# QueensGambit/CrazyAra

Measured on AMD Instinct MI355X. Metric: nn_evals_per_sec, higher is better.
Workload: dtype f16x3; 1 GPU; crazyhouse RISEv2 19-block (34x8x8 planes -> 5184 policy + value), batch=256, inputs resident in HBM, random-init seeded weights; batch=256, parallelism=replicas x1, precision=float16x3

## Files before the change

### crazyara_amd/csrc/nn/kernels.h

```cpp
#pragma once
#include <hip/hip_runtime.h>
#include <cstdint>

namespace cra {

typedef _Float16 half_t;

constexpr int kSquares = 64;

inline int64_t packed_weight_elems(int cout_pad, int k_total) { return int64_t(cout_pad) * k_total; }

struct ConvArgs {
    const void* x;
    const void* wpk;
    const void* wpk_lo;
    const float* bias;
    const void* resid;
    void* out;
    int batch;
    int cin;
    int cout_pad;
    int cout_real;
    int cout_ld;
    int ks;
    int relu;
    int out_policy_f32;
    int out_flat;
    int flat_pitch;
    int out_rows_f32;
    int rows_valid;
    float* softmax_out;
    const float* planes;
    int planes_c;
    int p8;
    float acc_scale;
    const void *pre_wpk, *pre_wpk_lo;
    const float* pre_bias;
    float pre_acc_scale;
    int dev;
    int few_boards;
    int x_ld;
};

template <typename T> void launch_conv_gemm(const ConvArgs& a, hipStream_t s);

struct BlockArgs {
    const void* x;
    void* y;
    const void* w1pk;
    const float* b1;
    const float* wdw;
    const float* b2;
    const void* w3pk;
    const void* w1pk_lo;
    const void* w3pk_lo;
    const float* b3;
    int batch, C, cop_pad, ks;
    const float* gate;
    float* pool_out;
    const float* dwpk;
};
template <typename T> void launch_block(const BlockArgs& a, hipStream_t s);
void launch_conv_gemm_x3(const ConvArgs& a, hipStream_t s);
void launch_block_x3(const BlockArgs& a, hipStream_t s);
void init_x3_kernel_attributes();
int block_x3_chunk_channels();
struct X3TowerBlock {
    const void *w1pk, *w1pk_lo, *w3pk, *w3pk_lo;
    const float* dwpk;
    const float* b3;
    const float* se_w1t;
    const float* se_w2t;
    const float* se_b;
    int cop_pad;
    int se_kind;
    float w1_inv, w3_scale, w3_inv;
};
struct X3TowerArgs {
    const float* x;
    float* y;
    const X3TowerBlock* blocks;
    int nblocks;
    int batch;
    int p8;
    int ks;
    int symmetric;
};
void launch_tower_x3(const X3TowerArgs& a, hipStream_t s);
struct X3SplitArgs {
    X3TowerBlock blk;
    const float* x_parts;
    float* y_parts;
    int gin;
    int batch, G;
    const float* pool_in;
    float* pool_out;
    int dev;
};
void launch_block_x3_split(const X3SplitArgs& a, hipStream_t s);
void launch_x3_split_finish(const float* parts, int gin, float* y, int batch, hipStream_t s);
template <typename T> void init_block_kernel_attributes();
template <typename T> int block_chunk_channels();

constexpr int kTowerWindow = 16;
struct TowerBlockDesc {
    const float* b3;
    const float* s3;
    const void* se_w1;
    const void* se_w2;
    const float* se_b;
    int cop_pad;
    int ks;
    int se_kind;
    float qx_inv, qt_inv, escale;
};
struct TowerArgs {
    const void* x;
    void* y;
    const TowerBlockDesc* blocks;
    const void* wstream;
    const float* bstream;
    const void* pstream;
    long long wstream_wave_frags, bstream_wave_floats, pstream_wave_bytes;
    int nblocks;
    int batch;
    const float* gate_in;
    float* pool_out;
    unsigned long long* trace;
// ... 144 lines not shown
```

### crazyara_amd/csrc/nn/rise_net.h

```cpp
#pragma once
#include <hip/hip_runtime.h>
#include <memory>
#include <string>
#include <utility>
#include <vector>

#include "netfile.h"

namespace cra {

struct RiseDesign {
    int batch = 0;
    int nb_input_channels = 0;
    int nb_policy = 0;
    int nb_aux = 0;
    int version = 0;
    int game_phase = 0;
    double flops_per_position = 0;
};

uint8_t float_to_e4m3(float v);
uint8_t float_to_e5m2(float v);

struct Precision {
// ... 36 lines not shown

    std::vector<std::pair<float, float>> calibration_maxima(const float* planes_host, int n_boards);

    float* d_planes() const { return d_planes_; }
    float* d_value() const { return d_value_; }
    float* d_probs() const { return d_probs_; }
    float* d_logits() const { return d_logits_; }
    void keep_logits(bool on);
    void* enable_block_dump(int* n_tiles);
    void dev_launch_op(int op, int iters);
    float* value_head_debug() const { return value_head_dbg_; }
    int dev_screen_prepare();
    long dev_screen_run(int op, int launches, long* words);
    std::string dev_screen_info(int op) const;
    float* d_aux() const { return d_aux_; }
    void forward_async();
    void launch_forward_in_stream();
    void forward_on(hipStream_t s);

    int launches_per_forward() const { return launches_; }
    const char* op_name(int i) const;
    void time_ops(int iters, float* ms);
    float time_forward(int iters);

    struct IoOverride {
        const float* planes = nullptr;
        float* value = nullptr;
        float* probs = nullptr;
        float* aux = nullptr;
    };
    bool last_submit_was_zero_copy() const { return last_zero_copy_; }

private:
    struct Impl;
    template <typename T> struct Builder;
    template <typename T> void build(const NetFile& nf);
    template <typename T> void enqueue(hipStream_t s, const IoOverride* io = nullptr);
    template <typename T> void launch_op(int i, hipStream_t s, const IoOverride* io = nullptr);
    void capture();
    bool buffers_are_pinned(const float* in_planes, float* value, float* probs, float* aux);
    bool last_zero_copy_ = false;
    bool counted_in_flight_ = false;
    int staged_calls_left_ = 0;
    struct DevSwitches {
        int conv_dev = -1;
        bool device_graph = false;
        bool lane_graph = false;
        bool lane_no_graph = false;
        bool predict_copy = false;
        bool predict_zero_copy = false;
        char lane_launches = 0;
        bool lane_sync = false;
        bool x3_symmetric = false;
        int x3_split_dev = 0;
        bool no_small_path = false;
        int small_conv_split = 2;
        bool own_stream = false;
        bool tower_trace = false;
        bool x3_value_one_launch;
        bool value_head_debug = false;
        int value_head_lds_pad = -1;
        int value_head_variant = 0;
        bool x3_no_head_chain = false;
        bool small_batch_heads_apart = false;
        DevSwitches();
    } dev_;
    float* value_head_dbg_ = nullptr;
    bool keep_logits_ = false;

    RiseDesign design_;
    std::string model_name_, model_file_path_;
    Precision prec_;
    std::vector<std::pair<float, float>> int8_calib_;
    static constexpr int kBoardSplitMaxBatch = 64;
    std::unique_ptr<RiseNet> small_;
    bool owns_stream_ = true;
    int stream_slot_ = -1;
    void touch_stream() const;
    std::string precision_arg_;
    int dyn_n_ = 0, dyn_prev_g_ = 1;
    bool small_path_ok() const;
    RiseNet& small_net();
    struct Turn;
    int cu_count_ = 256;
    int device_ = 0;
    int launches_ = 0;
    hipStream_t stream_ = nullptr;
    hipGraph_t graph_ = nullptr;
    hipGraphExec_t graph_exec_ = nullptr;
    void* d_desc_ = nullptr;
    float *d_planes_ = nullptr, *d_value_ = nullptr, *d_probs_ = nullptr, *d_logits_ = nullptr, *d_aux_ = nullptr;
    std::unique_ptr<Impl> impl_;
};

std::string int8_calibration_path(const std::string& model_file_path);
std::vector<std::pair<float, float>> read_int8_calibration(const std::string& model_file_path);
std::string calibrate_int8(const std::string& model_path, int device_id, const float* planes_host, int n_boards);
std::vector<float> default_calibration_planes(int channels, int version, int* n_boards);

}
```

### crazyara_amd/csrc/nn/rise_net.hip

```cpp
#include "rise_net.h"

#include <atomic>
#include <mutex>

#include <cmath>
#include <cstdio>
#include <cstdlib>
#include <cstring>
#include <fstream>
#include <type_traits>
#include <stdexcept>

#include "kernels.h"
#include "onnx_import.h"
#include "pack.h"
#include "../chess/planes_host.h"

namespace cra {

#define HIP_CHECK(expr)                                                                                      \
    do {                                                                                                     \
        hipError_t _e = (expr);                                                                              \
        if (_e != hipSuccess)                                                                                \
            throw std::runtime_error(std::string("HIP error ") + hipGetErrorString(_e) + " at " #expr);      \
// ... 24 lines not shown
    X3SplitArgs xs{};
    float* xs_y = nullptr;
};
}

struct ScreenOp {
    struct Buf { char* live; char* before; char* after; size_t bytes; };
    std::vector<Buf> writes;
    bool idempotent = true;
};

struct RiseNet::Impl {
    std::vector<void*> allocs;
    std::vector<std::pair<char*, size_t>> mutables;
    std::vector<Op> ops;
    std::vector<ScreenOp> screen;
    std::vector<void*> screen_allocs;
    unsigned* screen_bad = nullptr;
    int cin_pad = 0;

    void* dalloc(size_t bytes, bool constant = false) {
        void* p = nullptr;
        HIP_CHECK(hipMalloc(&p, bytes ? bytes : 16));
        allocs.push_back(p);
        if (!constant) mutables.emplace_back(static_cast<char*>(p), bytes ? bytes : 16);
        return p;
    }
    template <typename U> U* upload(const std::vector<U>& h) {
        U* d = static_cast<U*>(dalloc(h.size() * sizeof(U), true));
        HIP_CHECK(hipMemcpy(d, h.data(), h.size() * sizeof(U), hipMemcpyHostToDevice));
        return d;
    }
    float* upload_d2f(const std::vector<double>& h, size_t pad_to = 0) {
        std::vector<float> f(std::max(h.size(), pad_to), 0.f);
        for (size_t i = 0; i < h.size(); ++i) f[i] = float(h[i]);
        return upload(f);
    }
    ~Impl() {
        for (void* p : allocs) (void)hipFree(p);
        for (void* p : screen_allocs) (void)hipFree(p);
    }
};

RiseNet::DevSwitches::DevSwitches() {
    if (const char* e = getenv("CRA_X3_CONV_DEV")) conv_dev = atoi(e);
    device_graph = getenv("CRA_DEVICE_GRAPH") != nullptr;
    lane_graph = getenv("CRA_LANE_GRAPH") != nullptr;
    lane_no_graph = getenv("CRA_LANE_NO_GRAPH") != nullptr;
    predict_copy = getenv("CRA_PREDICT_COPY") != nullptr;
    predict_zero_copy = getenv("CRA_PREDICT_ZERO_COPY") != nullptr;
    if (const char* e = getenv("CRA_LANE_LAUNCHES")) lane_launches = e[0];
    lane_sync = getenv("CRA_LANE_SYNC") != nullptr;
    if (const char* e = getenv("CRA_X3_TOWER")) x3_symmetric = e[0] == 's';
    if (const char* e = getenv("CRA_X3_SPLIT_DEV")) x3_split_dev = atoi(e);
    no_small_path = getenv("CRA_NO_SMALL_PATH") != nullptr;
    own_stream = getenv("CRA_OWN_STREAM_PER_NET") != nullptr;
    if (const char* e = getenv("CRA_SMALL_BATCH_CONV_SPLIT")) small_conv_split = atoi(e);
    tower_trace = getenv("CRA_TOWER_TRACE") != nullptr;
    x3_value_one_launch = kX3ValueHeadOneLaunch;
    if (const char* e = getenv("CRA_X3_VALUE_HEAD")) x3_value_one_launch = e[0] == 'o';
    value_head_debug = getenv("CRA_VALUE_HEAD_DEBUG") != nullptr;
    if (const char* e = getenv("CRA_VALUE_HEAD_LDS_PAD")) value_head_lds_pad = atoi(e);
    if (const char* e = getenv("CRA_VALUE_HEAD_VARIANT")) value_head_variant = atoi(e);
    x3_no_head_chain = getenv("CRA_X3_NO_HEAD_CHAIN") != nullptr;
    small_batch_heads_apart = getenv("CRA_SMALL_BATCH_HEADS_APART") != nullptr;
}

namespace {
struct NetStreams {
    std::mutex mu;
    int n = 0;
    hipStream_t s[16] = {};
    std::atomic<uint64_t> last[16] = {};
};
NetStreams g_net_streams[64];
std::atomic<uint64_t> g_stream_tick{1};

int take_net_stream(int device, hipStream_t* out) {
    NetStreams& ns = g_net_streams[device];
    std::lock_guard<std::mutex> lk(ns.mu);
    if (ns.n == 0) {
        int n = 4;
        if (const char* e = getenv("GPU_MAX_HW_QUEUES")) n = atoi(e);
        n = n < 1 ? 1 : n > 16 ? 16 : n;
        for (int i = 0; i < n; ++i) HIP_CHECK(hipStreamCreateWithFlags(&ns.s[i], hipStreamNonBlocking));
        ns.n = n;
    }
    int best = 0;
    for (int i = 1; i < ns.n; ++i)
        if (ns.last[i].load(std::memory_order_relaxed) < ns.last[best].load(std::memory_order_relaxed)) best = i;
    ns.last[best].store(g_stream_tick.fetch_add(1, std::memory_order_relaxed), std::memory_order_relaxed);
    *out = ns.s[best];
    return best;
}
}

void RiseNet::touch_stream() const {
    if (stream_slot_ >= 0) g_net_streams[device_].last[stream_slot_].store(g_stream_tick.fetch_add(1, std::memory_order_relaxed), std::memory_order_relaxed);
}

static thread_local hipStream_t g_companion_stream = nullptr;
static thread_local int g_companion_slot = -1;

Precision parse_precision(const std::string& precision) {
    Precision v;
    std::string prec = precision;
// ... 94 lines not shown
    (void)hipSetDevice(device_);
    small_.reset();
    if (stream_) {
        (void)hipStreamSynchronize(stream_);
        if (owns_stream_ && stream_slot_ < 0) turns_forget_stream(device_, stream_);
    }
    if (graph_exec_) (void)hipGraphExecDestroy(graph_exec_);
    if (graph_) (void)hipGraphDestroy(graph_);
    impl_.reset();
    if (stream_ && owns_stream_ && stream_slot_ < 0) (void)hipStreamDestroy(stream_);
}

namespace {
enum class Family {
    Tower,
    X3Tower,
    X3Split,
    Fused,
    Layers,
    Transformer
};
struct BlockPlan {
    Family family;
    bool gate_in_kernel;
};
}

template <typename T> struct RiseNet::Builder {
    static constexpr bool kHalf = std::is_same<T, half_t>::value;
    RiseNet& net;
    Impl& im;
    const NetFile& nf;
    const Precision& prec;
    const DevSwitches& dev;
    int B = 0, cin = 0, C = 0, cv = 0, fc = 0, cp = 0, n_labels = 0, cin_pad = 0;
    bool wdl = false, policy_map = true, dense_blocks = false, a0_blocks = false, dense_se = false;
    bool transformers = false;
    std::vector<bool> ntb;
    std::vector<std::string> se_types;
    std::vector<int> cops, ks;
    bool tower_ok = false;
    bool x3_tower = false;
    bool x3_split = false;
    bool head_ok = false;
    T *x0 = nullptr, *cur = nullptr, *nxt = nullptr, *e = nullptr, *f = nullptr;
    float *se_pool = nullptr, *se_gate = nullptr;
    const float* pending_gate = nullptr;
    int prod_op = -1;
    double macs = 0;
    std::vector<TowerBlockDesc> tower_blocks;
    TowerStreams tower_streams;
    const float* tower_gate = nullptr;
    std::vector<X3TowerBlock> x3_blocks;
    int x3_run_ks = 3;
    float* split_parts[2] = {nullptr, nullptr};
    static constexpr int kSplitMaxG = 10;

    Builder(RiseNet& n, const NetFile& file) : net(n), im(*n.impl_), nf(file), prec(n.prec_), dev(n.dev_) {}
    void read_model();
    BlockPlan plan(size_t i) const;
    bool block_fused(int k) const { return prec.fused && C == 256 && !transformers && !(prec.x3() && k != 3); }
    void upload_dense(const void*& wpk, const void*& wpk_lo, const Folded& fd, int co, int ci, int k, int co_pad, int ci_pad);
    void set_conv_weights(ConvArgs& c, const Folded& fd, int co, int ci, int k, int co_pad, int ci_pad, bool p8 = false);
    ConvArgs& conv_op(const Folded& fd, const void* x, void* out, int ci, int ci_pad, int co, int k, int relu, bool p8 = false);
    void add_conv(const std::string& conv, const std::string& bn, const T* x, T* out, const T* resid, int ci, int ci_pad, int co, int k,
                  int relu, float* out_policy, bool p8 = false);
    Op se_op(const SEWeights& se);
    void add_se(Op op, bool consumer_fused);
    void stem();
    void dense_tower();
    void dense_layer_blocks();
    void bottleneck_blocks();
    void transformer_block(size_t i);
    void flush_tower();
    void flush_x3_run();
    void one_launch_head();
    void policy_head();
    void softmax();
    void value_head();
    void merge_heads_small();
    void merge_forward();
};

template <typename T> void RiseNet::Builder<T>::read_model() {
    B = net.design_.batch;
    cin = int(nf.num("nb_input_channels"));
    C = int(nf.num("channels", 256));
    const int cop_init = int(nf.num("channels_operating_init"));
    const int cexp = int(nf.num("channel_expansion"));
    cv = int(nf.num("channels_value_head", 8));
    fc = int(nf.num("value_fc_size", 256));
    cp = int(nf.num("channels_policy_head"));
    wdl = nf.num("use_wdl") != 0 && nf.num("use_plys_to_end") != 0;
    std::vector<std::string> kernels = nf.list("kernels");
    se_types = nf.list("se_types");
    if (kernels.empty() || kernels.size() != se_types.size()) throw std::runtime_error("kernels/se_types mismatch in model file");
    const std::string conv_block = nf.str("conv_block", "mobile_bottlekneck_res_block");
    a0_blocks = conv_block == "a0_res_block";
    dense_blocks = conv_block == "classical_res_block" || a0_blocks;
    if (!dense_blocks && conv_block != "mobile_bottlekneck_res_block") throw std::runtime_error("unsupported conv_block '" + conv_block + "'");
    if (dense_blocks)
        for (const std::string& t : se_types) dense_se |= !(t == "none" || t.empty());
    if (dense_blocks && (C % 64 != 0 || C > 512)) throw std::runtime_error("channels must be a multiple of 64 and <= 512");
    if (C % 32 != 0 || C > 512) throw std::runtime_error("channels must be a multiple of 32 and <= 512");
    if (fc > 256 && fc % 256 != 0) throw std::runtime_error("unsupported value_fc_size");

// ... 248 lines not shown
        const bool x3_family = bp.family == Family::X3Tower || bp.family == Family::X3Split;
        if (!x3_blocks.empty() && x3_run_ks != k) flush_x3_run();
        TowerBlockDesc td{};
        X3TowerBlock xb{};
        const SEWeights se = load_se(nf, p, se_types[i], C);
        if (se.kind && bp.gate_in_kernel && bp.family == Family::Tower) {
            const auto pk = pack_se_tower(se);
            td.se_kind = se.kind;
            td.se_w1 = im.upload(pk.first);
            if (se.kind == 1) td.se_w2 = im.upload(pk.second);
            else td.se_b = im.upload(se.b);
        } else if (se.kind && bp.gate_in_kernel) {
            const auto pk = pack_se_x3(se, C);
            xb.se_kind = se.kind;
            xb.se_w1t = im.upload(pk.first);
            if (se.kind == 1) xb.se_w2t = im.upload(pk.second);
            else xb.se_b = im.upload(se.b);
        } else if (se.kind) {
            add_se(se_op(se), bp.family == Family::Fused);
        }
        macs += se.macs;
        if (bp.family == Family::Tower) {
            if (prec.int8() && i >= net.int8_calib_.size()) throw std::runtime_error("INT8 calibration file holds fewer blocks than the model");
            const TowerBlockPack pk = pack_tower_block(fold_block(nf, p), C, cop, k, prec.int8() ? 2 : prec.fp8_tower() ? 1 : 0,
                                                       prec.int8() ? net.int8_calib_[i] : std::pair<float, float>{});
            if (!pk.s3.empty()) td.s3 = im.upload(pk.s3);
            td.b3 = im.upload(pk.b3);
            td.qx_inv = pk.qx_inv;
            td.qt_inv = pk.qt_inv;
            td.escale = pk.escale;
            td.cop_pad = round_up(cop, 128);
            td.ks = k;
            if (tower_blocks.empty()) {
                tower_gate = pending_gate;
                pending_gate = nullptr;
            }
            tower_blocks.push_back(td);
            tower_streams.append(pk.s);
        } else if (x3_family) {
            const int cop_pad = round_up(cop, block_x3_chunk_channels());
            const X3BlockPack pk = pack_x3_block(fold_block(nf, p), C, cop, k, cop_pad, prec.p8() && bp.family != Family::X3Split);
            xb.w1pk = im.upload(pk.w1.hi);
            xb.w1pk_lo = im.upload(pk.w1.lo);
            xb.w3pk = im.upload(pk.w3.hi);
            xb.w3pk_lo = im.upload(pk.w3.lo);
            xb.dwpk = im.upload(pk.dw);
            xb.b3 = im.upload(pk.b3);
            xb.w1_inv = float(pk.w1_inv);
            xb.w3_inv = float(pk.w3_inv);
            xb.w3_scale = float(1.0 / pk.w3_inv);
            xb.cop_pad = cop_pad;
            if (x3_blocks.empty()) x3_run_ks = k;
            x3_blocks.push_back(xb);
        } else if (bp.family == Family::Fused) {
            const int cop_pad = round_up(cop, prec.x3() ? block_x3_chunk_channels() : block_chunk_channels<T>());
            const BlockFold bf = fold_block(nf, p);
            Op op;
            op.kind = OpKind::Block;
            BlockArgs& ba = op.blk;
            ba.x = cur;
            ba.y = nxt;
            upload_dense(ba.w1pk, ba.w1pk_lo, bf.expand, cop, C, 1, cop_pad, C);
            upload_dense(ba.w3pk, ba.w3pk_lo, bf.project, C, cop, 1, C, cop_pad);
            ba.b1 = im.upload_d2f(bf.expand.b, cop_pad);
            ba.wdw = im.upload(pack_depthwise_taps(bf.dw, cop, k, cop_pad));
            ba.b2 = im.upload_d2f(bf.dw.b, cop_pad);
            ba.b3 = im.upload_d2f(bf.project.b, C);
            ba.batch = B;
            ba.C = C;
            ba.cop_pad = cop_pad;
            ba.ks = k;
            if (k == 3)
                ba.dwpk = im.upload(prec.x3() ? pack_x3_depthwise_records(bf.expand, bf.dw, cop, cop_pad, 3)
                                             : pack_depthwise_records12(bf.expand, bf.dw, cop, cop_pad));
            ba.gate = pending_gate;
            pending_gate = nullptr;
            prod_op = int(im.ops.size());
            im.ops.push_back(op);
            std::swap(cur, nxt);
        } else {
            add_conv(p + ".body.0", p + ".body.1", cur, e, nullptr, C, C, cop, 1, true, nullptr);
            {
                Folded fd = fold_bn(nf, p + ".body.3", p + ".body.4");
                Op op;
                op.kind = OpKind::Depthwise;
                op.x = e;
                op.y = f;
                op.w0 = im.upload(pack_depthwise_taps(fd, cop, k, cop));
                op.b0 = im.upload_d2f(fd.b);
                op.C = cop;
                op.ks = k;
                im.ops.push_back(op);
                macs += double(kSquares) * cop * k * k;
            }
            add_conv(p + ".body.6", p + ".body.7", f, nxt, cur, cop, cop, C, 1, false, nullptr);
            std::swap(cur, nxt);
            prod_op = -1;
            continue;
        }
        macs += double(kSquares) * cop * (2.0 * C + k * k);
    }
    flush_tower();
    flush_x3_run();
}

template <typename T> void RiseNet::Builder<T>::transformer_block(size_t i) {
// ... 14 lines not shown
        ConvArgs& c = conv_op(n.proj, f, xs, D, D, D, 1, 0);
        c.resid = xs;
        c.cout_ld = C;
    }
    {
        ConvArgs& c = conv_op(n.projection, xs, xs + D, D, D, M, 1, 0);
        c.x_ld = C;
        c.cout_ld = C;
    }
    conv_op(n.mhca, xs + D, f, M, M, M, 3, 1).x_ld = C;
    {
        ConvArgs& c = conv_op(n.mhca_proj, f, xs + D, M, M, M, 1, 0);
        c.resid = xs + D;
        c.cout_ld = C;
    }
    conv_op(n.mlp1, xs, e, C, C, H, 1, 1);
    conv_op(n.mlp2, e, cur, H, H, C, 1, 0).resid = xs;
    macs += n.macs;
    prod_op = -1;
}

template <typename T> void RiseNet::Builder<T>::flush_tower() {
    if (tower_blocks.empty()) return;
    Op op;
    op.kind = OpKind::Tower;
    op.tw.x = cur;
    op.tw.y = nxt;
    op.tw.blocks = im.upload(tower_blocks);
    op.tw.nblocks = int(tower_blocks.size());
    const TowerImage ti = close_tower_streams(std::move(tower_streams), prec.fp8_tower());
    tower_streams = TowerStreams();
    if (prec.fp8_tower()) {
        op.tw.fp8 = prec.int8() ? 2 : 1;
        op.tw.wstream_e_frags = ti.e_frags;
        op.tw.wstream = im.upload(ti.w8);
    } else {
        op.tw.wstream = im.upload(ti.w);
    }
    op.tw.bstream = im.upload(ti.b);
    op.tw.pstream = im.upload(ti.p);
    op.tw.wstream_wave_frags = ti.w_wave_frags;
    op.tw.bstream_wave_floats = ti.b_wave_floats;
    op.tw.pstream_wave_bytes = ti.p_wave_bytes;
    op.tw.batch = B;
    op.tw.gate_in = tower_gate;
    if (dev.tower_trace) op.tw.trace = static_cast<unsigned long long*>(im.dalloc(2 * 256 * sizeof(unsigned long long)));
    prod_op = int(im.ops.size());
    im.ops.push_back(op);
    tower_blocks.clear();
    tower_gate = nullptr;
    std::swap(cur, nxt);
}

template <typename T> void RiseNet::Builder<T>::flush_x3_run() {
    if (x3_blocks.empty()) return;
    if (x3_split && x3_run_ks == 3) {
        if (!split_parts[0])
            for (auto& q : split_parts) q = static_cast<float*>(im.dalloc(size_t(B) * kSplitMaxG * kSquares * C * sizeof(float)));
        const int max_g = std::max(1, std::min(int(kSplitMaxG), net.cu_count_ / B));
        const int nb = int(x3_blocks.size());
        int gin = 1;
        for (int k = 0; k < nb; ++k) {
            Op op;
            op.kind = OpKind::BlockX3Split;
            op.xs.blk = x3_blocks[k];
            op.xs.x_parts = k == 0 ? reinterpret_cast<const float*>(cur) : split_parts[k % 2];
            op.xs.y_parts = split_parts[(k + 1) % 2];
            op.xs.gin = gin;
            op.xs.batch = B;
            op.xs.G = std::min(max_g, x3_blocks[k].cop_pad / block_x3_chunk_channels());
            op.xs.dev = dev.x3_split_dev;
            if (k > 0 && x3_blocks[k].se_kind != 0 && !(dev.x3_split_dev & 8)) {
                float* pools = static_cast<float*>(im.dalloc(size_t(B) * kSplitMaxG * C * sizeof(float)));
                im.ops.back().xs.pool_out = pools;
                op.xs.pool_in = pools;
            }
            gin = op.xs.G;
            im.ops.push_back(op);
        }
        Op fin;
        fin.kind = OpKind::X3SplitFinish;
        fin.xs.x_parts = split_parts[nb % 2];
        fin.xs.gin = gin;
        fin.xs.batch = B;
        fin.xs_y = reinterpret_cast<float*>(nxt);
        im.ops.push_back(fin);
    } else {
        Op op;
        op.kind = OpKind::TowerX3;
        op.tx.x = reinterpret_cast<const float*>(cur);
        op.tx.y = reinterpret_cast<float*>(nxt);
        op.tx.blocks = im.upload(x3_blocks);
        op.tx.nblocks = int(x3_blocks.size());
        op.tx.batch = B;
        op.tx.p8 = prec.p8() ? 1 : 0;
        op.tx.ks = x3_run_ks;
        op.tx.symmetric = dev.x3_symmetric ? 1 : 0;
        im.ops.push_back(op);
    }
    x3_blocks.clear();
    prod_op = -1;
    std::swap(cur, nxt);
}

template <typename T> void RiseNet::Builder<T>::one_launch_head() {
    const Folded fv = fold_bn(nf, "value_head.body.0", "value_head.body.1");
    const HeadStreams hs = pack_head(fold_bn(nf, "policy_head.body.0", "policy_head.body.1"), fold_bn(nf, "policy_head.body.3", ""), fv, C, cv, cp);
    Op op;
    op.kind = OpKind::Head;
    HeadArgs& h = op.hd;
    h.x = cur;
    h.logits = net.d_logits_;
    h.probs = net.d_probs_;
    h.value = net.d_value_;
    h.aux = net.d_aux_;
    h.s1 = im.upload(hs.s1);
    h.b1 = im.upload(hs.b1);
    h.s2 = im.upload(hs.s2);
    h.s1_wave_frags = 9 * 16 + 16 + 16;
    h.s2_wave_frags = 18 * 3 + 9;
    h.vconv_bias = im.upload_d2f(fv.b, 8);
    h.cp = cp;
    h.batch = B;
    if (dev.tower_trace) h.trace = static_cast<unsigned long long*>(im.dalloc(64 * sizeof(unsigned long long)));
    const int nfl = kSquares * cv;
    if (wdl) {
        h.fc1_w = im.upload(pack_value_wdl(nf, nfl, 512));
        const float* bw = nf.get("value_head.body_wdl.0.bias").data;
        h.wdl_b[0] = bw[0]; h.wdl_b[1] = bw[1]; h.wdl_b[2] = bw[2];
        h.wdl_b[3] = nf.get("value_head.body_plys.0.bias").data[0];
        h.wdlp = 1;
        macs += 4.0 * nfl;
    } else {
        const TensorView& w2 = nf.get("value_head.body_final.2.weight");
        const float* bb = nf.get("value_head.body_final.0.bias").data;
        h.fc1_w = im.upload(pack_value_fc1_threads(nf, nfl, fc));
        h.fc1_b = im.upload(std::vector<float>(bb, bb + fc));
        h.fc2_w = im.upload(std::vector<float>(w2.data, w2.data + fc));
        h.fc2_b = nf.get("value_head.body_final.2.bias").data[0];
        macs += double(nfl) * fc + fc;
    }
    macs += double(kSquares) * 9 * (double(C) * C + double(C) * cp) + double(kSquares) * C * cv;
    im.ops.push_back(op);
}

template <typename T> void RiseNet::Builder<T>::policy_head() {
    const bool head_chain = prec.p8() && policy_map && C == 256 && round_up(cp, 16) <= 128 && !x3_split;
    const bool head_chain_x3 = prec.x3() && !prec.p8() && prec.fused && policy_map && C == 256 && round_up(cp, 16) <= 128 && !x3_split &&
                               !dev.x3_no_head_chain;
    if (head_chain || head_chain_x3) {
        Folded f1 = fold_bn(nf, "policy_head.body.0", "policy_head.body.1");
        double inv1 = 1.0;
        SplitPack s1 = head_chain ? pack_dense_p8(f1, C, C, 3, C, C, &inv1) : pack_dense_split(f1, C, C, 3, C, C);
// ... 889 lines not shown
```

### crazyara_amd/csrc/nn/x3.hip

```cpp
#include "kernels.h"
#include "device_utils.h"
#include "value_head_body.h"

#include <algorithm>
#include <cstdlib>
#include <stdexcept>
#include <type_traits>

#ifndef CRA_X3_ABL
#define CRA_X3_ABL 0
#endif
#ifndef X3_SGB_VALU
#define X3_SGB_VALU 10
#endif
#if CRA_X3_ABL != 0 && !defined(CRA_DEVELOPMENT)
#error "CRA_X3_ABL is a development switch (wrong results): build with -DCRA_DEVELOPMENT"
#endif
#if defined(CRA_X3_TRACE) && !defined(CRA_DEVELOPMENT)
#error "CRA_X3_TRACE is a development switch: build with -DCRA_DEVELOPMENT"
#endif

namespace cra {

#ifdef CRA_X3_TRACE
// ... 1532 lines not shown
    float* yb = a.y_parts + (size_t(b) * G_ + g) * 64 * C;
    f32x4 psum[NJ];
#pragma unroll
    for (int j = 0; j < NJ; ++j) psum[j] = f32x4{0.f, 0.f, 0.f, 0.f};
#pragma unroll
    for (int j = 0; j < NJ; ++j) {
        const int co0 = (wave * NJ + j) * 16 + lg * 4;
#pragma unroll
        for (int t = 0; t < 4; ++t) {
            const int sq = t * 16 + l15;
            f32x4 v = accP[j][t];
            if (g == 0) {
                float rh[4], rl[4];
                load4<half_t>(T.xh + sq * XROW + co0, rh);
                load4<half_t>(T.xl + sq * XROW + co0, rl);
#pragma unroll
                for (int r = 0; r < 4; ++r) v[r] += rh[r] + rl[r];
            }
            *reinterpret_cast<f32x4*>(yb + size_t(x3_square(sq)) * C + co0) = v;
            if (a.pool_out) {
#pragma unroll
                for (int r = 0; r < 4; ++r) psum[j][r] += v[r];
            }
        }
    }
    if (a.pool_out) {
        float* po = a.pool_out + (size_t(b) * G_ + g) * C;
#pragma unroll
        for (int j = 0; j < NJ; ++j) {
            float p[4] = {psum[j][0], psum[j][1], psum[j][2], psum[j][3]};
#pragma unroll
            for (int r = 0; r < 4; ++r) {
                p[r] += dpp_mov<0x111>(p[r]);
                p[r] += dpp_mov<0x112>(p[r]);
                p[r] += dpp_mov<0x114>(p[r]);
                p[r] += dpp_mov<0x118>(p[r]);
            }
            if (l15 == 15) *reinterpret_cast<f32x4*>(po + (wave * NJ + j) * 16 + lg * 4) = f32x4{p[0], p[1], p[2], p[3]};
        }
    }
}

__global__ __launch_bounds__(256) void x3_split_finish_kernel(const float* parts, int gin, float* y, int batch) {
    constexpr int per_board = 64 * X3Block::C / 4;
    for (int i = blockIdx.x * 256 + threadIdx.x; i < batch * per_board; i += gridDim.x * 256) {
        const int b = i / per_board, e = i - b * per_board;
        const f32x4* p = reinterpret_cast<const f32x4*>(parts + size_t(b) * gin * 64 * X3Block::C) + e;
        f32x4 s = p[0];
        for (int g = 1; g < gin; ++g) s += p[size_t(g) * per_board];
        reinterpret_cast<f32x4*>(y)[i] = s;
    }
}

template <int KS>
__global__ __launch_bounds__(512) void tower_x3_roles_kernel(const X3TowerArgs a) {
    static_assert(KS == 3 || KS == 5, "depthwise 3x3 or 5x5 (X3Depthwise / X3Depthwise5)");
    constexpr int REC = KS == 3 ? 256 : 512;
    using G = X3Block;
    static_assert(G::NE == 1 && G::T2BUF == 2 && G::CK == 128, "the role kernel uses the NE = 1 tile geometry (two t2 buffers of 128 channels)");
    constexpr int C = G::C, CK = G::CK, XROW = G::XROW, TROW = G::TROW;
    extern __shared__ __attribute__((aligned(16))) char smem[];
    const X3Tiles T = x3_tiles(smem);
    const int b = blockIdx.x;
    const int tid = threadIdx.x, lane = tid & 63, l15 = lane & 15, lg = lane >> 4;
    const int wave = __builtin_amdgcn_readfirstlane(tid >> 6);
    const bool expand_role = wave < 4;
    const int w = wave & 3;
    const uint32_t lane_off = uint32_t(lane) * 16u;
    x3_stage_tile(T, a.x + size_t(b) * 64 * C, nullptr, tid);
    __syncthreads();
#if defined(CRA_DEVELOPMENT) && defined(CRA_X3_EW)
    constexpr int EW = CRA_X3_EW;
#else
    constexpr int EW = 2;
#endif
    half8 e_h[EW][2], e_l[EW][2];
    bool first_chunk_requested = false;
    if (expand_role) {
    for (int blk = 0; blk < a.nblocks; ++blk) {
        const X3TowerBlock& d = a.blocks[blk];
        if (blk > 0 && d.se_kind != 0) {
            x3_se_phase(T, d, reinterpret_cast<float*>(T.t2h), tid);
            first_chunk_requested = false;
#pragma unroll
            for (int ne = 0; ne < 2; ++ne) {
#pragma unroll
                for (int q = 0; q < EW; ++q) { asm volatile("" : "=v"(e_h[q][ne])); asm volatile("" : "=v"(e_l[q][ne])); }
            }
        }
        const X3Weights W = x3_weights(d.w1pk, d.w1pk_lo, d.w3pk, d.w3pk_lo, d.dwpk, d.cop_pad);
        const int n = W.cop_pad / CK;
        const int nslab3 = W.cop_pad >> 5;
#ifdef CRA_X3_TRACE
        const bool tracing = (b == 0 || b == 131) && blk == CRA_X3_TRACE;
        int trace_n = 0;
#endif
        {
            const bool hi = l15 >= 8;
            const X3EdgeOffsets edge = x3_edge_offsets(l15);
            auto load_e = [&](int i, int s) {
                if constexpr (X3_ABL & 16) return;
#pragma unroll
                for (int ne = 0; ne < 2; ++ne) {
                    const uint32_t f = uint32_t(i * (CK / 16) + w * 2 + ne) * (C / 32) + uint32_t(s);
                    e_h[s % EW][ne] = x3_frag(W.w1h, lane_off, f);
                    e_l[s % EW][ne] = x3_frag(W.w1l, lane_off, f);
                }
            };
            auto load_first_chunk = [&](const X3Weights& Wx) {
                if constexpr (X3_ABL & 16) return;
#pragma unroll
                for (int s = 0; s < EW; ++s)
#pragma unroll
                    for (int ne = 0; ne < 2; ++ne) {
                        const uint32_t f = uint32_t(w * 2 + ne) * (C / 32) + uint32_t(s);
                        e_h[s][ne] = x3_frag(Wx.w1h, lane_off, f);
                        e_l[s][ne] = x3_frag(Wx.w1l, lane_off, f);
                    }
            };
            if constexpr (X3_ABL & 16) {
#pragma unroll
                for (int s = 0; s < EW; ++s)
#pragma unroll
                    for (int ne = 0; ne < 2; ++ne) e_h[s][ne] = e_l[s][ne] = *reinterpret_cast<const half8*>(T.xh + lane * 8);
            }
            if (!first_chunk_requested) load_first_chunk(W);
            float* const my_dws = T.dws + (w * 2) * REC;
            f32x4 accE[2][4], accD[2][4];
            X3Depthwise dw;
            X3Depthwise5 dw5;
            const X3EdgeOffsets5 edge5 = x3_edge_offsets5(l15);
            auto interval = [&](auto hase_c, auto hasd_c, int i) {
                constexpr bool HASE = decltype(hase_c)::value, HASD = decltype(hasd_c)::value;
                half8 ring_h[4], ring_l[4];
                auto read_step = [&](int st) {
                    if constexpr (X3_ABL & 8) {
                        ring_h[st % 4] = e_h[0][0];
                        ring_l[st % 4] = e_l[0][0];
                    } else {
                        ring_h[st % 4] = *reinterpret_cast<const half8*>(T.xh + ((st & 3) * 16 + l15) * XROW + (st >> 2) * 32 + lg * 8);
                        ring_l[st % 4] = *reinterpret_cast<const half8*>(T.xl + ((st & 3) * 16 + l15) * XROW + (st >> 2) * 32 + lg * 8);
                    }
                };
                f32x4 dw_raw[2][REC / 256];
                if constexpr (HASE) {
#pragma unroll
                    for (int ne = 0; ne < 2; ++ne)
#pragma unroll
                        for (int h2 = 0; h2 < REC / 256; ++h2)
                            dw_raw[ne][h2] = __builtin_bit_cast(f32x4, __builtin_amdgcn_raw_buffer_load_b128(W.dw, lane_off, uint32_t(i * CK + (w * 2 + ne) * 16) * uint32_t(REC / 4) + uint32_t(h2) * 1024u, 0));
#pragma unroll
                    for (int ne = 0; ne < 2; ++ne)
#pragma unroll
                        for (int t = 0; t < 4; ++t) accE[ne][t] = f32x4{0.f, 0.f, 0.f, 0.f};
                    read_step(0); read_step(1); read_step(2);
                }
                if constexpr (HASD && KS == 3) dw.template load<0>(my_dws, lg, edge);
                half_t* const t2h = T.t2h + ((i - 1) & 1) * 64 * TROW;
                half_t* const t2l = T.t2l + ((i - 1) & 1) * 64 * TROW;
#pragma unroll
                for (int sl = 0; sl < C / 32; ++sl) {
                    const int dt = sl / 4, ph = sl % 4;
                    if constexpr (HASD) {
                        if constexpr (KS == 3) {
                            if (ph == 2) dw.template load<1>(my_dws + dt * 256, lg, edge);
                            if (sl == 4) dw.template load<0>(my_dws + 256, lg, edge);
                        } else {
                            if (ph == 0) dw5.template load<0>(my_dws + dt * REC, lg, edge5);
                            if (ph == 1) dw5.template load<1>(my_dws + dt * REC, lg, edge5);
                            if (ph == 2) dw5.template load<2>(my_dws + dt * REC, lg, edge5);
                            if (ph == 3) dw5.template load<3>(my_dws + dt * REC, lg, edge5);
                        }
                    }
                    __builtin_amdgcn_sched_barrier(0);
                    if constexpr (HASE) {
#pragma unroll
                        for (int t = 0; t < 4; ++t) {
                            const int st = sl * 4 + t;
                            if (st + 3 < 4 * (C / 32)) read_step(st + 3);
#pragma unroll
                            for (int ne = 0; ne < 2; ++ne) {
                                if constexpr ((X3_ABL & 128) != 0) {
                                    x3_mfma(e_h[sl % EW][ne], ring_h[st % 4], accE[ne][t], true);
                                    if (sl & 1) x3_mfma8(x3_cat(e_l[0][ne], e_l[1][ne]), x3_cat(ring_l[st % 4], ring_l[(st + 1) % 4]), accE[ne][t], true);
                                    continue;
                                }
                                x3_mfma(e_l[sl % EW][ne], ring_h[st % 4], accE[ne][t], !(X3_ABL & 2));
                                x3_mfma(e_h[sl % EW][ne], ring_l[st % 4], accE[ne][t], !(X3_ABL & 2));
                                x3_mfma(e_h[sl % EW][ne], ring_h[st % 4], accE[ne][t], !(X3_ABL & 2));
                            }
                        }
                        if (sl + EW < C / 32) load_e(i, sl + EW);
                        else load_e(i + 1 < n ? i + 1 : i, sl + EW - C / 32);
                    }
                    if constexpr (HASD) {
                        if constexpr (KS == 3) {
                            if (ph == 0) dw.template gather<0>(accD[dt], hi);
                            if (ph == 1) { dw.template taps<0>(0, 4); dw.pin_taps(0, 4, 0); }
                            if (ph == 2) dw.template gather<1>(accD[dt], hi);
                        } else {
                            if (ph == 0) { dw5.template gather<0>(accD[dt], hi, 1.f); dw5.template taps<0>(); }
                            if (ph == 1) { dw5.template gather<1>(accD[dt], hi, 1.f); dw5.template taps<1>(); }
                            if (ph == 2) { dw5.template gather<2>(accD[dt], hi, 1.f); dw5.template taps<2>(); }
                            if (ph == 3) { dw5.template gather<3>(accD[dt], hi, 1.f); dw5.template taps<3>(); }
                        }
                        if (ph == 3) {
                            if constexpr (KS == 3) dw.template taps<1>(0, 4);
                            const int cl = (w * 2 + dt) * 16 + lg * 4;
#pragma unroll
                            for (int t = 0; t < 4; ++t) {
                                half4 h, l;
                                split4(KS == 3 ? dw.outv[t] : dw5.outv[t], h, l);
                                if constexpr (X3_ABL & 64) {
                                    asm volatile("" ::"v"(h), "v"(l));
                                } else {
                                    *reinterpret_cast<half4*>(t2h + (t * 16 + l15) * TROW + cl) = h;
                                    *reinterpret_cast<half4*>(t2l + (t * 16 + l15) * TROW + cl) = l;
                                }
                            }
                        }
                    }
                    if constexpr (HASE && HASD) {
#pragma unroll
                        for (int r = 0; r < 24; ++r) {
                            __builtin_amdgcn_sched_group_barrier(0x008, 1, 0);
                            __builtin_amdgcn_sched_group_barrier(0x002, 4, 0);
                        }
                    }
                    __builtin_amdgcn_sched_barrier(0);
                }
                if constexpr (HASE) {
#pragma unroll
                    for (int ne = 0; ne < 2; ++ne)
#pragma unroll
                        for (int h2 = 0; h2 < REC / 256; ++h2) *reinterpret_cast<f32x4*>(my_dws + ne * REC + h2 * 256 + lane * 4) = dw_raw[ne][h2];
#pragma unroll
                    for (int ne = 0; ne < 2; ++ne)
#pragma unroll
                        for (int t = 0; t < 4; ++t) accD[ne][t] = accE[ne][t];
                }
            };
            for (int i = 0; i <= n; ++i) {
                const int kk = i - 1;
                X3_STAMP(0);
                if (i == 0) interval(std::true_type{}, std::false_type{}, i);
                else if (i < n) interval(std::true_type{}, std::true_type{}, i);
                else interval(std::false_type{}, std::true_type{}, i);
                X3_STAMP(3);
                if constexpr (!(X3_ABL & 32)) __syncthreads();
                X3_STAMP(4);
            }
            first_chunk_requested = false;
            if (blk + 1 < a.nblocks && a.blocks[blk + 1].se_kind == 0) {
                const X3TowerBlock& dn = a.blocks[blk + 1];
                load_first_chunk(x3_weights(dn.w1pk, dn.w1pk_lo, dn.w3pk, dn.w3pk_lo, dn.dwpk, dn.cop_pad));
                first_chunk_requested = true;
            }
            __syncthreads();
            { const int kk = n; X3_STAMP(5); }
        }
    }
    } else {
    for (int blk = 0; blk < a.nblocks; ++blk) {
        const X3TowerBlock& d = a.blocks[blk];
        if (blk > 0 && d.se_kind != 0) x3_se_phase(T, d, reinterpret_cast<float*>(T.t2h), tid);
        const X3Weights W = x3_weights(d.w1pk, d.w1pk_lo, d.w3pk, d.w3pk_lo, d.dwpk, d.cop_pad);
        const int n = W.cop_pad / CK;
        const int nslab3 = W.cop_pad >> 5;
#ifdef CRA_X3_TRACE
        const bool tracing = (b == 0 || b == 131) && blk == CRA_X3_TRACE;
        int trace_n = 0;
#endif
        {
#if defined(CRA_DEVELOPMENT) && defined(CRA_X3_PW)
            constexpr int PW = CRA_X3_PW, NJ = 4;
#else
            constexpr int PW = 2, NJ = 4;
#endif
            half8 p_h[PW][NJ], p_l[PW][NJ];
            auto load_p = [&](int k, int s2) {
                if constexpr (X3_ABL & 16) return;
#pragma unroll
                for (int j = 0; j < NJ; ++j) {
                    const uint32_t f = uint32_t(w * NJ + j) * uint32_t(nslab3) + uint32_t(k * (CK / 32) + s2);
                    p_h[s2 % PW][j] = x3_frag(W.w3h, lane_off, f);
                    p_l[s2 % PW][j] = x3_frag(W.w3l, lane_off, f);
                }
            };
            if constexpr (X3_ABL & 16) {
#pragma unroll
                for (int s2 = 0; s2 < PW; ++s2)
#pragma unroll
                    for (int j = 0; j < NJ; ++j) p_h[s2][j] = p_l[s2][j] = *reinterpret_cast<const half8*>(T.xl + lane * 8);
            }
            f32x4 accP[NJ][4];
#pragma unroll
            for (int j = 0; j < NJ; ++j) {
                const f32x4 bs = *reinterpret_cast<const f32x4*>(d.b3 + (w * NJ + j) * 16 + lg * 4);
#pragma unroll
                for (int t = 0; t < 4; ++t) accP[j][t] = bs;
            }
#pragma unroll
            for (int s2 = 0; s2 < PW; ++s2) load_p(0, s2);
            if constexpr (!(X3_ABL & 32)) {
                __syncthreads();
                __syncthreads();
            }
            for (int kk = 0; kk < n; ++kk) {
                const half_t* const t2h = T.t2h + (kk & 1) * 64 * TROW;
                const half_t* const t2l = T.t2l + (kk & 1) * 64 * TROW;
                X3_STAMP(8);
                half8 bh[2][4], bl[2][4];
                auto read_t2 = [&](int s2, half8 (&h)[4], half8 (&l)[4]) {
#pragma unroll
                    for (int t = 0; t < 4; ++t) {
                        if constexpr (X3_ABL & 8) {
                            h[t] = p_h[s2 % PW][0];
                            l[t] = p_l[s2 % PW][0];
                        } else {
                            h[t] = *reinterpret_cast<const half8*>(t2h + (t * 16 + l15) * TROW + s2 * 32 + lg * 8);
                            l[t] = *reinterpret_cast<const half8*>(t2l + (t * 16 + l15) * TROW + s2 * 32 + lg * 8);
                        }
                    }
                };
                read_t2(0, bh[0], bl[0]);
#pragma unroll
                for (int s2 = 0; s2 < CK / 32; ++s2) {
                    if (s2 + 1 < CK / 32) read_t2(s2 + 1, bh[(s2 + 1) & 1], bl[(s2 + 1) & 1]);
                    __builtin_amdgcn_sched_barrier(0);
#pragma unroll
                    for (int j = 0; j < NJ; ++j)
#pragma unroll
                        for (int t = 0; t < 4; ++t) x3_mfma(p_l[s2 % PW][j], bh[s2 & 1][t], accP[j][t], !(X3_ABL & 4));
#pragma unroll
                    for (int j = 0; j < NJ; ++j)
#pragma unroll
                        for (int t = 0; t < 4; ++t) x3_mfma(p_h[s2 % PW][j], bl[s2 & 1][t], accP[j][t], !(X3_ABL & 4));
#pragma unroll
                    for (int j = 0; j < NJ; ++j)
#pragma unroll
                        for (int t = 0; t < 4; ++t) x3_mfma(p_h[s2 % PW][j], bh[s2 & 1][t], accP[j][t], !(X3_ABL & 4));
                    if (s2 + PW < CK / 32) load_p(kk, s2 + PW);
                    else load_p(kk + 1 < n ? kk + 1 : kk, s2 + PW - CK / 32);
                    if (s2 == 1) X3_STAMP(9);
                    __builtin_amdgcn_sched_barrier(0);
                }
                X3_STAMP(10);
                if (kk + 1 < n) {
                    if constexpr (!(X3_ABL & 32)) __syncthreads();
                }
                X3_STAMP(11);
            }
#pragma unroll
            for (int j = 0; j < NJ; ++j) {
                const int co0 = (w * NJ + j) * 16 + lg * 4;
#pragma unroll
                for (int t = 0; t < 4; ++t) {
                    const int sq = t * 16 + l15;
                    float rh[4], rl[4], v[4];
                    load4<half_t>(T.xh + sq * XROW + co0, rh);
                    load4<half_t>(T.xl + sq * XROW + co0, rl);
#pragma unroll
                    for (int r = 0; r < 4; ++r) v[r] = accP[j][t][r] + (rh[r] + rl[r]);
                    half4 h, l;
                    split4(v, h, l);
                    *reinterpret_cast<half4*>(T.xh + sq * XROW + co0) = h;
                    *reinterpret_cast<half4*>(T.xl + sq * XROW + co0) = l;
                }
            }
            { const int kk = n; X3_STAMP(12); }
            __syncthreads();
            { const int kk = n; X3_STAMP(13); }
        }
    }
    }
    float* yb = a.y + size_t(b) * 64 * C;
#pragma unroll 1
    for (int i = tid; i < 64 * (C / 8); i += G::NTHR) {
        const int sq = i / (C / 8), v = i - sq * (C / 8), r = x3_row(sq);
        float fh[8], fl[8];
        load8<half_t>(T.xh + r * XROW + v * 8, fh);
        load8<half_t>(T.xl + r * XROW + v * 8, fl);
#pragma unroll
        for (int j = 0; j < 8; ++j) fh[j] += fl[j];
        store8<float>(yb + size_t(sq) * C + v * 8, fh);
    }
}

namespace {
__device__ __forceinline__ void x3_se_gate_from_mean(const X3TowerBlock& d, float* scratch, int tid) {
    constexpr int GRP = 36;
    float* se_mean = scratch;
    float* se_h = scratch + 8 * GRP;
    float* se_gate = se_h + 4 * GRP;
    f32x4 wa[16], wb[16];
    auto load_thread_weights = [&](const float* base, f32x4 (&dst)[16]) {
        const f32x4* pk = reinterpret_cast<const f32x4*>(base) + tid;
#pragma unroll
        for (int i = 0; i < 16; ++i) dst[i] = pk[i * 512];
    };
    load_thread_weights(d.se_w1t, wa);
    load_thread_weights(d.se_kind == 1 ? d.se_w2t : d.se_w1t + size_t(16) * 512 * 4, wb);
    __syncthreads();
    auto dot32 = [](const f32x4 (&w)[16], const float* v, float& s0, float& s1) {
#pragma unroll
// ... 482 lines not shown
```

Baseline: 331,500 evals/s.

## Skip padded half of last 128-channel chunk in x3 tower blocks

Adds a per-block bitmask marking blocks whose expanded channel count only half-fills the last 128-wide chunk. For those blocks the fused float16x3 tower kernel runs the final expand, depthwise and projection intervals at 64-channel width, so the MFMA work and weight loads on zero padding are skipped. Templated interval and projection lambdas take compile-time widths. This adds code-size and scheduling complexity, and a risk of misindexed loads for the half-width prefetch. CRA_X3_CHUNKS=pad restores the old behaviour.

```diff
diff --git a/crazyara_amd/csrc/nn/kernels.h b/crazyara_amd/csrc/nn/kernels.h
--- a/crazyara_amd/csrc/nn/kernels.h
+++ b/crazyara_amd/csrc/nn/kernels.h
@@ -74,6 +74,7 @@
     const float* se_b;
     int cop_pad;
     int se_kind;
+    int half_chunks;
     float w1_inv, w3_scale, w3_inv;
 };
 struct X3TowerArgs {
diff --git a/crazyara_amd/csrc/nn/rise_net.h b/crazyara_amd/csrc/nn/rise_net.h
--- a/crazyara_amd/csrc/nn/rise_net.h
+++ b/crazyara_amd/csrc/nn/rise_net.h
@@ -112,6 +112,7 @@
         char lane_launches = 0;
         bool lane_sync = false;
         bool x3_symmetric = false;
+        bool x3_chunks_pad = false;
         int x3_split_dev = 0;
         bool no_small_path = false;
         int small_conv_split = 2;
diff --git a/crazyara_amd/csrc/nn/rise_net.hip b/crazyara_amd/csrc/nn/rise_net.hip
--- a/crazyara_amd/csrc/nn/rise_net.hip
+++ b/crazyara_amd/csrc/nn/rise_net.hip
@@ -100,6 +100,10 @@
     if (const char* e = getenv("CRA_LANE_LAUNCHES")) lane_launches = e[0];
     lane_sync = getenv("CRA_LANE_SYNC") != nullptr;
     if (const char* e = getenv("CRA_X3_TOWER")) x3_symmetric = e[0] == 's';
+    if (const char* e = getenv("CRA_X3_CHUNKS")) {
+        if (std::string(e) != "pad" && std::string(e) != "tail") throw std::invalid_argument("CRA_X3_CHUNKS: pad or tail");
+        x3_chunks_pad = e[0] == 'p';
+    }
     if (const char* e = getenv("CRA_X3_SPLIT_DEV")) x3_split_dev = atoi(e);
     no_small_path = getenv("CRA_NO_SMALL_PATH") != nullptr;
     own_stream = getenv("CRA_OWN_STREAM_PER_NET") != nullptr;
@@ -300,6 +304,7 @@
     TowerStreams tower_streams;
     const float* tower_gate = nullptr;
     std::vector<X3TowerBlock> x3_blocks;
+    std::vector<int> x3_cops;
     int x3_run_ks = 3;
     float* split_parts[2] = {nullptr, nullptr};
     static constexpr int kSplitMaxG = 10;
@@ -654,6 +659,7 @@
             xb.cop_pad = cop_pad;
             if (x3_blocks.empty()) x3_run_ks = k;
             x3_blocks.push_back(xb);
+            x3_cops.push_back(cop);
         } else if (bp.family == Family::Fused) {
             const int cop_pad = round_up(cop, prec.x3() ? block_x3_chunk_channels() : block_chunk_channels<T>());
             const BlockFold bf = fold_block(nf, p);
@@ -774,6 +780,12 @@
     std::swap(cur, nxt);
 }
 
+static int x3_chunk_schedule(int cop, int cop_pad) {
+    const int n = cop_pad / 128;
+    if (n > 31) throw std::invalid_argument("float16x3 tower: more than 31 chunks of 128 expanded channels");
+    return n >= 2 && (cop + 63) / 64 % 2 == 1 ? 1 << (n - 1) : 0;
+}
+
 template <typename T> void RiseNet::Builder<T>::flush_x3_run() {
     if (x3_blocks.empty()) return;
     if (x3_split && x3_run_ks == 3) {
@@ -812,15 +824,18 @@
         op.kind = OpKind::TowerX3;
         op.tx.x = reinterpret_cast<const float*>(cur);
         op.tx.y = reinterpret_cast<float*>(nxt);
-        op.tx.blocks = im.upload(x3_blocks);
-        op.tx.nblocks = int(x3_blocks.size());
         op.tx.batch = B;
         op.tx.p8 = prec.p8() ? 1 : 0;
         op.tx.ks = x3_run_ks;
         op.tx.symmetric = dev.x3_symmetric ? 1 : 0;
+        if (!op.tx.p8 && op.tx.ks == 3 && !op.tx.symmetric && !dev.x3_chunks_pad)
+            for (size_t k = 0; k < x3_blocks.size(); ++k) x3_blocks[k].half_chunks = x3_chunk_schedule(x3_cops[k], x3_blocks[k].cop_pad);
+        op.tx.blocks = im.upload(x3_blocks);
+        op.tx.nblocks = int(x3_blocks.size());
         im.ops.push_back(op);
     }
     x3_blocks.clear();
+    x3_cops.clear();
     prod_op = -1;
     std::swap(cur, nxt);
 }
diff --git a/crazyara_amd/csrc/nn/x3.hip b/crazyara_amd/csrc/nn/x3.hip
--- a/crazyara_amd/csrc/nn/x3.hip
+++ b/crazyara_amd/csrc/nn/x3.hip
@@ -1608,6 +1608,9 @@
     }
 }
 
+__device__ __forceinline__ bool x3_tail_chunk(const X3TowerBlock& d, int n) {
+    return (uint32_t(__builtin_amdgcn_readfirstlane(d.half_chunks)) >> (n - 1)) & 1u;
+}
 template <int KS>
 __global__ __launch_bounds__(512) void tower_x3_roles_kernel(const X3TowerArgs a) {
     static_assert(KS == 3 || KS == 5, "depthwise 3x3 or 5x5 (X3Depthwise / X3Depthwise5)");
@@ -1647,6 +1650,7 @@
         const X3Weights W = x3_weights(d.w1pk, d.w1pk_lo, d.w3pk, d.w3pk_lo, d.dwpk, d.cop_pad);
         const int n = W.cop_pad / CK;
         const int nslab3 = W.cop_pad >> 5;
+        const bool tail = KS == 3 && x3_tail_chunk(d, n);
 #ifdef CRA_X3_TRACE
         const bool tracing = (b == 0 || b == 131) && blk == CRA_X3_TRACE;
         int trace_n = 0;
@@ -1654,11 +1658,11 @@
         {
             const bool hi = l15 >= 8;
             const X3EdgeOffsets edge = x3_edge_offsets(l15);
-            auto load_e = [&](int i, int s) {
+            auto load_e = [&](auto nt_c, int i, bool half, int s) {
                 if constexpr (X3_ABL & 16) return;
 #pragma unroll
-                for (int ne = 0; ne < 2; ++ne) {
-                    const uint32_t f = uint32_t(i * (CK / 16) + w * 2 + ne) * (C / 32) + uint32_t(s);
+                for (int ne = 0; ne < decltype(nt_c)::value; ++ne) {
+                    const uint32_t f = uint32_t(i * (CK / 16) + (half ? w : w * 2 + ne)) * (C / 32) + uint32_t(s);
                     e_h[s % EW][ne] = x3_frag(W.w1h, lane_off, f);
                     e_l[s % EW][ne] = x3_frag(W.w1l, lane_off, f);
                 }
@@ -1686,8 +1690,10 @@
             X3Depthwise dw;
             X3Depthwise5 dw5;
             const X3EdgeOffsets5 edge5 = x3_edge_offsets5(l15);
-            auto interval = [&](auto hase_c, auto hasd_c, int i) {
-                constexpr bool HASE = decltype(hase_c)::value, HASD = decltype(hasd_c)::value;
+            auto interval = [&](auto ewid_c, auto dwid_c, int i) {
+                constexpr int EWID = decltype(ewid_c)::value, DWID = decltype(dwid_c)::value;
+                constexpr bool HASE = EWID != 0, HASD = DWID != 0;
+                constexpr int NE = EWID / 64, NDT = DWID / 64;
                 half8 ring_h[4], ring_l[4];
                 auto read_step = [&](int st) {
                     if constexpr (X3_ABL & 8) {
@@ -1701,12 +1707,12 @@
                 f32x4 dw_raw[2][REC / 256];
                 if constexpr (HASE) {
 #pragma unroll
-                    for (int ne = 0; ne < 2; ++ne)
+                    for (int ne = 0; ne < NE; ++ne)
 #pragma unroll
                         for (int h2 = 0; h2 < REC / 256; ++h2)
-                            dw_raw[ne][h2] = __builtin_bit_cast(f32x4, __builtin_amdgcn_raw_buffer_load_b128(W.dw, lane_off, uint32_t(i * CK + (w * 2 + ne) * 16) * uint32_t(REC / 4) + uint32_t(h2) * 1024u, 0));
-#pragma unroll
-                    for (int ne = 0; ne < 2; ++ne)
+                            dw_raw[ne][h2] = __builtin_bit_cast(f32x4, __builtin_amdgcn_raw_buffer_load_b128(W.dw, lane_off, uint32_t(i * CK + (NE == 2 ? w * 2 + ne : w) * 16) * uint32_t(REC / 4) + uint32_t(h2) * 1024u, 0));
+#pragma unroll
+                    for (int ne = 0; ne < NE; ++ne)
 #pragma unroll
                         for (int t = 0; t < 4; ++t) accE[ne][t] = f32x4{0.f, 0.f, 0.f, 0.f};
                     read_step(0); read_step(1); read_step(2);
@@ -1717,7 +1723,8 @@
 #pragma unroll
                 for (int sl = 0; sl < C / 32; ++sl) {
                     const int dt = sl / 4, ph = sl % 4;
-                    if constexpr (HASD) {
+                    const bool dwork = HASD && dt < NDT;
+                    if (dwork) {
                         if constexpr (KS == 3) {
                             if (ph == 2) dw.template load<1>(my_dws + dt * 256, lg, edge);
                             if (sl == 4) dw.template load<0>(my_dws + 256, lg, edge);
@@ -1735,7 +1742,7 @@
                             const int st = sl * 4 + t;
                             if (st + 3 < 4 * (C / 32)) read_step(st + 3);
 #pragma unroll
-                            for (int ne = 0; ne < 2; ++ne) {
+                            for (int ne = 0; ne < NE; ++ne) {
                                 if constexpr ((X3_ABL & 128) != 0) {
                                     x3_mfma(e_h[sl % EW][ne], ring_h[st % 4], accE[ne][t], true);
                                     if (sl & 1) x3_mfma8(x3_cat(e_l[0][ne], e_l[1][ne]), x3_cat(ring_l[st % 4], ring_l[(st + 1) % 4]), accE[ne][t], true);
@@ -1746,10 +1753,11 @@
                                 x3_mfma(e_h[sl % EW][ne], ring_h[st % 4], accE[ne][t], !(X3_ABL & 2));
                             }
                         }
-                        if (sl + EW < C / 32) load_e(i, sl + EW);
-                        else load_e(i + 1 < n ? i + 1 : i, sl + EW - C / 32);
+                        if (sl + EW < C / 32) load_e(std::integral_constant<int, NE>{}, i, NE == 1, sl + EW);
+                        else if (i + 1 < n) load_e(std::integral_constant<int, 2>{}, i + 1, tail && i + 2 == n, sl + EW - C / 32);
+                        else load_e(std::integral_constant<int, NE>{}, i, NE == 1, sl + EW - C / 32);
                     }
-                    if constexpr (HASD) {
+                    if (dwork) {
                         if constexpr (KS == 3) {
                             if (ph == 0) dw.template gather<0>(accD[dt], hi);
                             if (ph == 1) { dw.template taps<0>(0, 4); dw.pin_taps(0, 4, 0); }
@@ -1762,7 +1770,7 @@
                         }
                         if (ph == 3) {
                             if constexpr (KS == 3) dw.template taps<1>(0, 4);
-                            const int cl = (w * 2 + dt) * 16 + lg * 4;
+                            const int cl = (NDT == 2 ? w * 2 + dt : w) * 16 + lg * 4;
 #pragma unroll
                             for (int t = 0; t < 4; ++t) {
                                 half4 h, l;
@@ -1777,35 +1785,46 @@
                         }
                     }
                     if constexpr (HASE && HASD) {
-#pragma unroll
-                        for (int r = 0; r < 24; ++r) {
-                            __builtin_amdgcn_sched_group_barrier(0x008, 1, 0);
-                            __builtin_amdgcn_sched_group_barrier(0x002, 4, 0);
+                        if (dwork) {
+                            constexpr int NV = NE == 2 ? 4 : 8;
+#pragma unroll
+                            for (int r = 0; r < 12 * NE; ++r) {
+                                __builtin_amdgcn_sched_group_barrier(0x008, 1, 0);
+                                __builtin_amdgcn_sched_group_barrier(0x002, NV, 0);
+                            }
                         }
                     }
                     __builtin_amdgcn_sched_barrier(0);
                 }
                 if constexpr (HASE) {
 #pragma unroll
-                    for (int ne = 0; ne < 2; ++ne)
+                    for (int ne = 0; ne < NE; ++ne)
 #pragma unroll
                         for (int h2 = 0; h2 < REC / 256; ++h2) *reinterpret_cast<f32x4*>(my_dws + ne * REC + h2 * 256 + lane * 4) = dw_raw[ne][h2];
 #pragma unroll
-                    for (int ne = 0; ne < 2; ++ne)
+                    for (int ne = 0; ne < NE; ++ne)
 #pragma unroll
                         for (int t = 0; t < 4; ++t) accD[ne][t] = accE[ne][t];
                 }
             };
-            for (int i = 0; i <= n; ++i) {
+            auto step = [&](auto ewid_c, auto dwid_c, int i) {
                 const int kk = i - 1;
                 X3_STAMP(0);
-                if (i == 0) interval(std::true_type{}, std::false_type{}, i);
-                else if (i < n) interval(std::true_type{}, std::true_type{}, i);
-                else interval(std::false_type{}, std::true_type{}, i);
+                interval(ewid_c, dwid_c, i);
                 X3_STAMP(3);
                 if constexpr (!(X3_ABL & 32)) __syncthreads();
                 X3_STAMP(4);
-            }
+            };
+            using W0 = std::integral_constant<int, 0>;
+            using W64 = std::integral_constant<int, 64>;
+            using W128 = std::integral_constant<int, 128>;
+            const int nfull = tail ? n - 1 : n;
+            step(W128{}, W0{}, 0);
+            for (int i = 1; i < nfull; ++i) step(W128{}, W128{}, i);
+            if (tail) {
+                step(W64{}, W128{}, n - 1);
+                step(W0{}, W64{}, n);
+            } else step(W0{}, W128{}, n);
             first_chunk_requested = false;
             if (blk + 1 < a.nblocks && a.blocks[blk + 1].se_kind == 0) {
                 const X3TowerBlock& dn = a.blocks[blk + 1];
@@ -1823,6 +1842,7 @@
         const X3Weights W = x3_weights(d.w1pk, d.w1pk_lo, d.w3pk, d.w3pk_lo, d.dwpk, d.cop_pad);
         const int n = W.cop_pad / CK;
         const int nslab3 = W.cop_pad >> 5;
+        const bool tail = KS == 3 && x3_tail_chunk(d, n);
 #ifdef CRA_X3_TRACE
         const bool tracing = (b == 0 || b == 131) && blk == CRA_X3_TRACE;
         int trace_n = 0;
@@ -1862,7 +1882,8 @@
                 __syncthreads();
                 __syncthreads();
             }
-            for (int kk = 0; kk < n; ++kk) {
+            auto project = [&](auto pwid_c, int kk) {
+                constexpr int NS = decltype(pwid_c)::value / 32;
                 const half_t* const t2h = T.t2h + (kk & 1) * 64 * TROW;
                 const half_t* const t2l = T.t2l + (kk & 1) * 64 * TROW;
                 X3_STAMP(8);
@@ -1881,8 +1902,8 @@
                 };
                 read_t2(0, bh[0], bl[0]);
 #pragma unroll
-                for (int s2 = 0; s2 < CK / 32; ++s2) {
-                    if (s2 + 1 < CK / 32) read_t2(s2 + 1, bh[(s2 + 1) & 1], bl[(s2 + 1) & 1]);
+                for (int s2 = 0; s2 < NS; ++s2) {
+                    if (s2 + 1 < NS) read_t2(s2 + 1, bh[(s2 + 1) & 1], bl[(s2 + 1) & 1]);
                     __builtin_amdgcn_sched_barrier(0);
 #pragma unroll
                     for (int j = 0; j < NJ; ++j)
@@ -1896,8 +1917,8 @@
                     for (int j = 0; j < NJ; ++j)
 #pragma unroll
                         for (int t = 0; t < 4; ++t) x3_mfma(p_h[s2 % PW][j], bh[s2 & 1][t], accP[j][t], !(X3_ABL & 4));
-                    if (s2 + PW < CK / 32) load_p(kk, s2 + PW);
-                    else load_p(kk + 1 < n ? kk + 1 : kk, s2 + PW - CK / 32);
+                    if (s2 + PW < NS) load_p(kk, s2 + PW);
+                    else load_p(kk + 1 < n ? kk + 1 : kk, s2 + PW - NS);
                     if (s2 == 1) X3_STAMP(9);
                     __builtin_amdgcn_sched_barrier(0);
                 }
@@ -1906,7 +1927,9 @@
                     if constexpr (!(X3_ABL & 32)) __syncthreads();
                 }
                 X3_STAMP(11);
-            }
+            };
+            for (int kk = 0; kk < (tail ? n - 1 : n); ++kk) project(std::integral_constant<int, CK>{}, kk);
+            if (tail) project(std::integral_constant<int, 64>{}, n - 1);
 #pragma unroll
             for (int j = 0; j < NJ; ++j) {
                 const int co0 = (w * NJ + j) * 16 + lg * 4;
```

Measured after the change: 337,400 evals/s, median of 6. 1.02x the previous value.
